# seungju-k1m/Distributed_RL

Hardware: NVIDIA H100
Metric: learner transitions/sec (sample+target+prio-update) (higher is better)
Workload: dtype f32

## Files before the change

distributed_rl_b200/csrc/common.cuh:

```cuda
#pragma once
#include <cuda_runtime.h>
#include <stdint.h>
#include <stdio.h>
#include <string.h>
#include <atomic>

#include "../../include/b2rl.h"

namespace b2rl {

void set_error(const char* fmt, ...);
extern std::atomic<int64_t> g_launches;
inline void count_launch(int n = 1) { g_launches.fetch_add(n, std::memory_order_relaxed); }

#define B2RL_CUDA(call)                                                              \
  do {                                                                               \
    cudaError_t e_ = (call);                                                         \
    if (e_ != cudaSuccess) {                                                         \
      b2rl::set_error("%s:%d %s -> %s", __FILE__, __LINE__, #call, cudaGetErrorString(e_)); \
      return B2RL_ERR_CUDA;                                                          \
    }                                                                                \
  } while (0)

#define B2RL_CHECK_LAUNCH()                                                          \
  do {                                                                               \
    cudaError_t e_ = cudaGetLastError();                                             \
    if (e_ != cudaSuccess) {                                                         \
      b2rl::set_error("%s:%d kernel launch -> %s", __FILE__, __LINE__, cudaGetErrorString(e_)); \
      return B2RL_ERR_CUDA;                                                          \
    }                                                                                \
  } while (0)

#define B2RL_REQUIRE(cond, msg)                                                      \
  do {                                                                               \
    if (!(cond)) {                                                                   \
      b2rl::set_error("%s:%d invalid argument: %s", __FILE__, __LINE__, msg);        \
      return B2RL_ERR_INVALID;                                                       \
    }                                                                                \
  } while (0)

struct DeviceGuard {
  int prev = -1;
  bool ok = true;
  explicit DeviceGuard(int dev) {
    if (cudaGetDevice(&prev) != cudaSuccess) { ok = false; return; }
    if (prev != dev && cudaSetDevice(dev) != cudaSuccess) ok = false;
    target = dev;
  }
  ~DeviceGuard() {
    if (prev >= 0 && prev != target) cudaSetDevice(prev);
  }
  int target = -1;
};

inline cudaError_t sm_count(int dev, int* out) {
  static int sms[64] = {0};
  if (!sms[dev & 63]) {
    const cudaError_t e = cudaDeviceGetAttribute(&sms[dev & 63], cudaDevAttrMultiProcessorCount, dev);
    if (e != cudaSuccess) return e;
  }
  *out = sms[dev & 63];
  return cudaSuccess;
}

template <auto K>
cudaError_t set_max_dynamic_smem(int dev, size_t bytes) {
  static bool done[64] = {false};
  if (done[dev & 63]) return cudaSuccess;
  const cudaError_t e = cudaFuncSetAttribute(K, cudaFuncAttributeMaxDynamicSharedMemorySize, (int)bytes);
  if (e == cudaSuccess) done[dev & 63] = true;
  return e;
}


__device__ __forceinline__ float powcr(float x, float e) {
  return (float)pow((double)x, (double)e);
}

__host__ __device__ __forceinline__ uint32_t lowbias32(uint32_t x) {
  x ^= x >> 16; x *= 0x7feb352dU; x ^= x >> 15; x *= 0x846ca68bU; x ^= x >> 16;
  return x;
}

__host__ __device__ __forceinline__ void philox4x32_10(uint64_t ctr, uint64_t seed, uint32_t out[4]) {
  uint32_t c0 = (uint32_t)ctr, c1 = (uint32_t)(ctr >> 32), c2 = 0u, c3 = 0u;
  uint32_t k0 = (uint32_t)seed, k1 = (uint32_t)(seed >> 32);
#pragma unroll
  for (int r = 0; r < 10; ++r) {
    uint64_t p0 = (uint64_t)0xD2511F53U * c0;
    uint64_t p1 = (uint64_t)0xCD9E8D57U * c2;
    uint32_t n0 = (uint32_t)(p1 >> 32) ^ c1 ^ k0;
    uint32_t n1 = (uint32_t)p1;
    uint32_t n2 = (uint32_t)(p0 >> 32) ^ c3 ^ k1;
    uint32_t n3 = (uint32_t)p0;
    c0 = n0; c1 = n1; c2 = n2; c3 = n3;
// ... 76 lines not shown
```

distributed_rl_b200/csrc/conv1.cu:

```cuda
#include "common.cuh"
#include "frames.cuh"
#include "hopper.cuh"

namespace b2rl {
namespace conv1 {

using namespace sm90;

constexpr int C_IN = 4, HW = 84, KS = 8, STRIDE = 4, OHW = 20;
constexpr int C_OUT_MAX = 32;
constexpr int K_TOTAL = C_IN * KS * KS;
constexpr int POS = OHW * OHW;
constexpr int TILE_M = 128;
constexpr int TILES = (POS + TILE_M - 1) / TILE_M;
constexpr int NSPLIT = 4;
constexpr int A_STAGES = 2;
constexpr int A_TILE_BYTES = TILE_M * K_TOTAL;
constexpr int A_CHUNK_BYTES = TILE_M * 128;
constexpr int RAW_STRIDE = 28288;
constexpr int CONSUMERS = 256, PRODUCERS = 256;
constexpr int THREADS = CONSUMERS + PRODUCERS + 32;

__host__ __device__ __forceinline__ int sw128_offset(int rows, int n, int k) {
  const int j = k >> 7, kk = k & 127;
// ... 47 lines not shown
struct Params {
  FrameSource src;
  const int64_t* idx;
  int64_t n;
  const int8_t* bq;
  const float* scale;
  float* out;
  int relu;
};

template <int N> struct Acc;
template <> struct Acc<128> {
  int32_t d[64];
  __device__ __forceinline__ void mma(uint64_t a, uint64_t b, uint32_t acc) { mma_u8s8_n128(d, a, b, acc); }
};
template <> struct Acc<64> {
  int32_t d[32];
  __device__ __forceinline__ void mma(uint64_t a, uint64_t b, uint32_t acc) { mma_u8s8_n64(d, a, b, acc); }
};

template <int N_NETS, int C_OUT, FrameKind KIND>
__global__ void __launch_bounds__(THREADS, 1)
k_conv1_fused(const __grid_constant__ Params P) {
  constexpr int N_PER_NET = NSPLIT * C_OUT;
  constexpr int N_TOTAL = N_NETS * N_PER_NET;
  constexpr int B_BYTES = N_TOTAL * K_TOTAL;
  extern __shared__ __align__(1024) uint8_t smem_raw[];
  uint8_t* smem = smem_raw + ((1024u - (sptr(smem_raw) & 1023u)) & 1023u);
  uint8_t* sB = smem;
  uint8_t* sA = smem + B_BYTES;
  uint8_t* sRaw = sA + A_STAGES * A_TILE_BYTES;
  __shared__ __align__(8) uint64_t b_full, raw_full[2], raw_empty[2], a_full[A_STAGES], a_empty[A_STAGES];
  __shared__ float s_scale[2 * C_OUT_MAX];
  if (threadIdx.x < N_NETS * C_OUT) s_scale[threadIdx.x] = P.scale[threadIdx.x] * (1.0f / 128.0f);

  const int warp = threadIdx.x >> 5, lane = threadIdx.x & 31;
  if (threadIdx.x == 0) {
    mbar_init(&b_full, 1);
    for (int i = 0; i < 2; ++i) { mbar_init(&raw_full[i], 1); mbar_init(&raw_empty[i], PRODUCERS); }
    for (int i = 0; i < A_STAGES; ++i) { mbar_init(&a_full[i], PRODUCERS); mbar_init(&a_empty[i], CONSUMERS); }
    mbar_init_fence();
  }
  __syncthreads();
  const int64_t units = P.n * TILES;
  const int64_t u0 = units * blockIdx.x / gridDim.x, u1 = units * (blockIdx.x + 1) / gridDim.x;
  const int64_t k_first = u0 / TILES, k_end = (u1 + TILES - 1) / TILES;

  if (warp == (CONSUMERS + PRODUCERS) / 32) {
    if (lane == 0) {
      const uint8_t* frames = frame_base<KIND>(P.src);
      mbar_expect_tx(&b_full, B_BYTES);
      constexpr int LOAD_CHUNK = (B_BYTES < 32768) ? B_BYTES : 32768;
      for (int off = 0; off < B_BYTES; off += LOAD_CHUNK) bulk_g2s(sB + off, P.bq + off, LOAD_CHUNK, &b_full);
      int it = 0;
      for (int64_t k = k_first; k < k_end; ++k, ++it) {
        const int s = it & 1;
        mbar_wait(&raw_empty[s], ((it >> 1) & 1) ^ 1);
        int64_t row = P.idx ? P.idx[k] : k;
        row = row < 0 ? 0 : (row >= P.src.rows ? P.src.rows - 1 : row);
        load_row<KIND>(P.src, frames, row, sRaw + s * RAW_STRIDE, &raw_full[s]);
      }
    }
  } else if (warp >= CONSUMERS / 32) {
    const int pt = threadIdx.x - CONSUMERS;
    const int r_local = pt & (TILE_M - 1);
    const int chalf = pt >> 7;
    int at = 0, it = 0;
    for (int64_t k = k_first; k < k_end; ++k, ++it) {
      const int s = it & 1;
      mbar_wait(&raw_full[s], (it >> 1) & 1);
      const uint8_t* raw = sRaw + s * RAW_STRIDE;
      const int t_lo = (int)max((int64_t)0, u0 - k * TILES), t_hi = (int)min((int64_t)TILES, u1 - k * TILES);
      for (int t = t_lo; t < t_hi; ++t, ++at) {
        const int stage = at % A_STAGES;
        mbar_wait(&a_empty[stage], ((at / A_STAGES) & 1) ^ 1);
// ... 99 lines not shown
  conv1::k_conv1_pack<<<c_out, conv1::K_TOTAL, 0, (cudaStream_t)stream>>>(w_dev, net, n_nets, c_out, bq_out_dev,
                                                                         scale_out_dev);
  count_launch();
  B2RL_CHECK_LAUNCH();
  return B2RL_OK;
}

extern "C" int b2rl_conv1_pack_jobs(const float* const* w_dev, const int32_t* net, const int32_t* n_nets,
                                    int8_t* const* bq_out_dev, float* const* scale_out_dev, int32_t jobs,
                                    int32_t c_out, void* stream) {
  B2RL_REQUIRE(w_dev && net && n_nets && bq_out_dev && scale_out_dev, "null argument");
  B2RL_REQUIRE(jobs >= 1 && jobs <= conv1::MAX_PACK_JOBS, "1..4 pack jobs");
  B2RL_REQUIRE(c_out == 16 || c_out == 32, "c_out must be 16 or 32");
  conv1::PackJobs J{};
  for (int j = 0; j < jobs; ++j) {
    B2RL_REQUIRE(w_dev[j] && bq_out_dev[j] && scale_out_dev[j], "null pack job");
    B2RL_REQUIRE(n_nets[j] >= 1 && n_nets[j] <= 2 && net[j] >= 0 && net[j] < n_nets[j], "n_nets must be 1 or 2");
    J.w[j] = w_dev[j]; J.bq[j] = bq_out_dev[j]; J.scale[j] = scale_out_dev[j];
    J.net[j] = net[j]; J.n_nets[j] = n_nets[j];
  }
  conv1::k_conv1_pack_jobs<<<dim3(c_out, jobs), conv1::K_TOTAL, 0, (cudaStream_t)stream>>>(J, c_out);
  count_launch();
  B2RL_CHECK_LAUNCH();
  return B2RL_OK;
}

template <int N_NETS, int C_OUT, FrameKind KIND>
static cudaError_t conv1_launch(const conv1::Params& P, unsigned grid, cudaStream_t st) {
  int dev = 0;
  cudaError_t e = cudaGetDevice(&dev);
  if (e == cudaSuccess)
    e = set_max_dynamic_smem<conv1::k_conv1_fused<N_NETS, C_OUT, KIND>>(dev, conv1::smem_bytes<N_NETS, C_OUT>());
  if (e != cudaSuccess) return e;
  conv1::k_conv1_fused<N_NETS, C_OUT, KIND><<<grid, conv1::THREADS, conv1::smem_bytes<N_NETS, C_OUT>(), st>>>(P);
  return cudaSuccess;
}

extern "C" int b2rl_conv1_fused(const b2rl_frames* frames, const int64_t* idx_dev, int64_t n, const int8_t* bq_dev,
                                const float* scale_dev, int32_t n_nets, int32_t c_out, float* out_dev, int32_t relu,
                                void* stream) {
  B2RL_REQUIRE(n >= 0, "negative n");
  conv1::Params P{};
  FrameKind kind;
  if (const int rc = check_frames(frames, P.src, kind)) return rc;
  if (n == 0) return B2RL_OK;
  B2RL_REQUIRE(bq_dev && scale_dev && out_dev, "null argument");
  B2RL_REQUIRE(n_nets == 1 || n_nets == 2, "n_nets must be 1 or 2");
  B2RL_REQUIRE(c_out == 16 || c_out == 32, "c_out must be 16 or 32");
  B2RL_REQUIRE(((uintptr_t)bq_dev % 16 == 0) && ((uintptr_t)out_dev % 16 == 0),
               "packed weights and output must be 16-byte aligned");
  int dev = 0;
  B2RL_CUDA(cudaGetDevice(&dev));
  int sms = 0;
  B2RL_CUDA(sm_count(dev, &sms));
  P.idx = idx_dev, P.n = n, P.bq = bq_dev, P.scale = scale_dev, P.out = out_dev, P.relu = relu;
  const int64_t units = n * conv1::TILES;
  const unsigned grid = (unsigned)((units < sms) ? units : sms);
  cudaStream_t st = (cudaStream_t)stream;
  const cudaError_t e = with_frame_kind(kind, [&](auto K) {
    constexpr FrameKind KIND = decltype(K)::value;
    if (c_out == 32) return n_nets == 1 ? conv1_launch<1, 32, KIND>(P, grid, st) : conv1_launch<2, 32, KIND>(P, grid, st);
    return n_nets == 1 ? conv1_launch<1, 16, KIND>(P, grid, st) : conv1_launch<2, 16, KIND>(P, grid, st);
  });
  B2RL_CUDA(e);
  count_launch();
  B2RL_CHECK_LAUNCH();
  return B2RL_OK;
}
```

distributed_rl_b200/csrc/dueling.cu:

```cuda
#include "common.cuh"

namespace b2rl {
namespace dueling {

constexpr int MAX_A = 32, MAX_H = 1024, ROWS_PER_CTA = 4;

__device__ __forceinline__ void load_weights(float* s_w, const float* __restrict__ wa, const float* __restrict__ wv,
                                             int A, int H) {
  const int na = (A * H) >> 2, nv = H >> 2;
  for (int i = threadIdx.x; i < na; i += blockDim.x)
    reinterpret_cast<float4*>(s_w)[i] = reinterpret_cast<const float4*>(wa)[i];
  for (int i = threadIdx.x; i < nv; i += blockDim.x)
    reinterpret_cast<float4*>(s_w + A * H)[i] = reinterpret_cast<const float4*>(wv)[i];
}

__device__ __forceinline__ float warp_sum(float v) {
#pragma unroll
  for (int o = 16; o > 0; o >>= 1) v = __fadd_rn(v, __shfl_xor_sync(0xffffffffu, v, o));
  return v;
}

constexpr int STAGE_UNROLL = 8;

template <int A_MAX>
__global__ void __launch_bounds__(ROWS_PER_CTA * 32)
k_dueling_forward(const float* __restrict__ h, int splits, int64_t split_stride, int M, int H,
                  const float* __restrict__ wa, int A, const float* __restrict__ wv, float* __restrict__ q,
                  float* __restrict__ h_out) {
  extern __shared__ float s_w[];
  float* s_h = s_w + A * H + H;
  load_weights(s_w, wa, wv, A, H);
  {
    const int m0 = blockIdx.x * ROWS_PER_CTA;
// ... 35 lines not shown
  float s[A_MAX], val = 0.0f;
#pragma unroll
  for (int j = 0; j < A_MAX; ++j) s[j] = 0.0f;
  for (int k = lane; k < H; k += 32) {
    const float ra = fmaxf(hr[k], 0.0f), rv = fmaxf(hr[H + k], 0.0f);
    val = __fmaf_rn(rv, s_w[A * H + k], val);
#pragma unroll
    for (int j = 0; j < A_MAX; ++j)
      if (j < A) s[j] = __fmaf_rn(ra, s_w[j * H + k], s[j]);
  }
#pragma unroll
  for (int o = 16; o > 0; o >>= 1) {
    val = __fadd_rn(val, __shfl_xor_sync(0xffffffffu, val, o));
#pragma unroll
    for (int j = 0; j < A_MAX; ++j)
      if (j < A) s[j] = __fadd_rn(s[j], __shfl_xor_sync(0xffffffffu, s[j], o));
  }
  float mine = 0.0f, total = 0.0f;
#pragma unroll
  for (int j = 0; j < A_MAX; ++j) {
    if (j < A) {
      total = __fadd_rn(total, s[j]);
      if (lane == j) mine = s[j];
    }
  }
  if (lane < A) q[(int64_t)m * A + lane] = __fsub_rn(__fadd_rn(mine, val), __fdiv_rn(total, (float)A));
}

__global__ void __launch_bounds__(ROWS_PER_CTA * 32)
k_dueling_backward_h(const float* __restrict__ h, const float* __restrict__ gq, int M, int H,
                     const float* __restrict__ wa, int A, const float* __restrict__ wv, float* __restrict__ gh,
                     float* __restrict__ ga) {
  extern __shared__ float s_w[];
  load_weights(s_w, wa, wv, A, H);
  __syncthreads();
  const int lane = threadIdx.x & 31, m = blockIdx.x * ROWS_PER_CTA + (threadIdx.x >> 5);
  if (m >= M) return;
  const float g = (lane < A) ? gq[(int64_t)m * A + lane] : 0.0f;
  const float gval = warp_sum(g);
  const float gadv = __fsub_rn(g, __fdiv_rn(gval, (float)A));
  if (lane < A) ga[(int64_t)m * (A + 1) + lane] = gadv;
  if (lane == 0) ga[(int64_t)m * (A + 1) + A] = gval;
  if (gh == nullptr) return;
  const float* hr = h + (int64_t)m * 2 * H;
  float* gr = gh + (int64_t)m * 2 * H;
  const int n = H >> 5;
  float ha[MAX_H / 32], hv[MAX_H / 32], s[MAX_H / 32];
#pragma unroll
  for (int i = 0; i < MAX_H / 32; ++i) {
    ha[i] = (i < n) ? hr[lane + 32 * i] : 0.0f;
    hv[i] = (i < n) ? hr[H + lane + 32 * i] : 0.0f;
    s[i] = 0.0f;
  }
  for (int j = 0; j < A; ++j) {
    const float gj = __shfl_sync(0xffffffffu, gadv, j);
#pragma unroll
    for (int i = 0; i < MAX_H / 32; ++i)
      if (i < n) s[i] = __fmaf_rn(gj, s_w[j * H + lane + 32 * i], s[i]);
  }
#pragma unroll
  for (int i = 0; i < MAX_H / 32; ++i) {
    if (i < n) {
      gr[lane + 32 * i] = ha[i] > 0.0f ? s[i] : 0.0f;
      gr[H + lane + 32 * i] = hv[i] > 0.0f ? __fmul_rn(gval, s_w[A * H + lane + 32 * i]) : 0.0f;
    }
  }
// ... 86 lines not shown
  if (A <= 8) {
    B2RL_CUDA(dueling_smem((const void*)dueling::k_dueling_forward<8>, smem));
    dueling::k_dueling_forward<8><<<grid, block, smem, st>>>(h_dev, splits, split_stride, (int)M, (int)H, wa_dev,
                                                                 (int)A, wv_dev, q_dev, h_out_dev);
  } else if (A <= 16) {
    B2RL_CUDA(dueling_smem((const void*)dueling::k_dueling_forward<16>, smem));
    dueling::k_dueling_forward<16><<<grid, block, smem, st>>>(h_dev, splits, split_stride, (int)M, (int)H, wa_dev,
                                                                 (int)A, wv_dev, q_dev, h_out_dev);
  } else {
    B2RL_CUDA(dueling_smem((const void*)dueling::k_dueling_forward<32>, smem));
    dueling::k_dueling_forward<32><<<grid, block, smem, st>>>(h_dev, splits, split_stride, (int)M, (int)H, wa_dev,
                                                                 (int)A, wv_dev, q_dev, h_out_dev);
  }
  count_launch();
  B2RL_CHECK_LAUNCH();
  return B2RL_OK;
}

extern "C" int b2rl_dueling_backward_w(const float* h_dev, const float* row_ws_dev, int64_t M, int64_t H, int64_t A,
                                       float* gwa_dev, float* gwv_dev, void* stream);

extern "C" int b2rl_dueling_backward(const float* h_dev, const float* gq_dev, int64_t M, int64_t H,
                                     const float* wa_dev, int64_t A, const float* wv_dev, float* gh_dev,
                                     float* gwa_dev, float* gwv_dev, float* row_ws_dev, void* stream) {
  if (int rc = dueling_check(h_dev, M, H, A)) return rc;
  B2RL_REQUIRE(gq_dev && wa_dev && wv_dev && row_ws_dev, "null argument");
  B2RL_REQUIRE(((uintptr_t)wa_dev % 16) == 0 && ((uintptr_t)wv_dev % 16) == 0, "weights must be 16-byte aligned");
  B2RL_REQUIRE((gwa_dev == nullptr) == (gwv_dev == nullptr), "both weight gradients or neither");
  cudaStream_t st = (cudaStream_t)stream;
  {
    const size_t smem = (size_t)(A + 1) * H * sizeof(float);
    B2RL_CUDA(dueling_smem((const void*)dueling::k_dueling_backward_h, smem));
    const unsigned grid = (unsigned)((M + dueling::ROWS_PER_CTA - 1) / dueling::ROWS_PER_CTA);
    dueling::k_dueling_backward_h<<<grid, dueling::ROWS_PER_CTA * 32, smem, st>>>(h_dev, gq_dev, (int)M, (int)H, wa_dev,
                                                                                 (int)A, wv_dev, gh_dev, row_ws_dev);
    count_launch();
    B2RL_CHECK_LAUNCH();
  }
  if (gwa_dev) return b2rl_dueling_backward_w(h_dev, row_ws_dev, M, H, A, gwa_dev, gwv_dev, stream);
  return B2RL_OK;
}

extern "C" int b2rl_dueling_backward_w(const float* h_dev, const float* row_ws_dev, int64_t M, int64_t H, int64_t A,
                                       float* gwa_dev, float* gwv_dev, void* stream) {
  if (int rc = dueling_check(h_dev, M, H, A)) return rc;
  B2RL_REQUIRE(row_ws_dev && gwa_dev && gwv_dev, "null argument");
  cudaStream_t st = (cudaStream_t)stream;
  {
    const unsigned grid = (unsigned)(2 * H / 8);
    if (A <= 8)
      dueling::k_dueling_backward_w<8><<<grid, 256, 0, st>>>(h_dev, row_ws_dev, (int)M, (int)H, (int)A, gwa_dev, gwv_dev);
    else if (A <= 16)
      dueling::k_dueling_backward_w<16><<<grid, 256, 0, st>>>(h_dev, row_ws_dev, (int)M, (int)H, (int)A, gwa_dev, gwv_dev);
    else
      dueling::k_dueling_backward_w<32><<<grid, 256, 0, st>>>(h_dev, row_ws_dev, (int)M, (int)H, (int)A, gwa_dev, gwv_dev);
    count_launch();
    B2RL_CHECK_LAUNCH();
  }
  return B2RL_OK;
}
```

distributed_rl_b200/csrc/hopper.cuh:

```cuda
#pragma once
#include <stdint.h>

namespace b2rl {
namespace sm90 {

__device__ __forceinline__ uint32_t sptr(const void* p) { return (uint32_t)__cvta_generic_to_shared(p); }
__device__ __forceinline__ void mbar_init(uint64_t* b, uint32_t c) {
  asm volatile("mbarrier.init.shared::cta.b64 [%0], %1;" ::"r"(sptr(b)), "r"(c));
}
__device__ __forceinline__ void mbar_init_fence() {
  asm volatile("fence.mbarrier_init.release.cluster;" ::: "memory");
  asm volatile("fence.proxy.async.shared::cta;" ::: "memory");
}
__device__ __forceinline__ void mbar_expect_tx(uint64_t* b, uint32_t bytes) {
  asm volatile("mbarrier.arrive.expect_tx.shared::cta.b64 _, [%0], %1;" ::"r"(sptr(b)), "r"(bytes) : "memory");
}
__device__ __forceinline__ void mbar_arrive(uint64_t* b) {
  asm volatile("mbarrier.arrive.shared::cta.b64 _, [%0];" ::"r"(sptr(b)) : "memory");
}
__device__ __forceinline__ void mbar_wait(uint64_t* b, uint32_t parity) {
  asm volatile(
      "{\n\t.reg .pred p;\n\t"
      "W_%=:\n\t"
      "mbarrier.try_wait.parity.shared::cta.b64 p, [%0], %1;\n\t"
      "@p bra D_%=;\n\t"
      "bra W_%=;\n\t"
      "D_%=:\n\t}" ::"r"(sptr(b)), "r"(parity) : "memory");
}
__device__ __forceinline__ void bulk_g2s(void* dst, const void* src, uint32_t bytes, uint64_t* bar) {
  asm volatile("cp.async.bulk.shared::cluster.global.mbarrier::complete_tx::bytes [%0], [%1], %2, [%3];" ::"r"(
                   sptr(dst)), "l"(src), "r"(bytes), "r"(sptr(bar)) : "memory");
}
__device__ __forceinline__ void bulk_s2g(void* dst, const void* src, uint32_t bytes) {
  asm volatile("cp.async.bulk.global.shared::cta.bulk_group [%0], [%1], %2;" ::"l"(dst), "r"(sptr(src)), "r"(bytes)
               : "memory");
}
__device__ __forceinline__ void bulk_commit() { asm volatile("cp.async.bulk.commit_group;" ::: "memory"); }
template <int N>
__device__ __forceinline__ void bulk_wait_read() { asm volatile("cp.async.bulk.wait_group.read %0;" ::"n"(N) : "memory"); }
__device__ __forceinline__ void bulk_wait_all() { asm volatile("cp.async.bulk.wait_group 0;" ::: "memory"); }
__device__ __forceinline__ void fence_async_smem() { asm volatile("fence.proxy.async.shared::cta;" ::: "memory"); }
__device__ __forceinline__ void named_sync(int id, int threads) {
  asm volatile("bar.sync %0, %1;" ::"r"(id), "r"(threads) : "memory");
}

__device__ __forceinline__ uint64_t make_desc(uint32_t smem_addr) {
  return (uint64_t)((smem_addr & 0x3FFFFu) >> 4) | (1ull << 16) | ((uint64_t)(1024 >> 4) << 32) | (1ull << 62);
}

__device__ __forceinline__ void wg_fence() { asm volatile("wgmma.fence.sync.aligned;" ::: "memory"); }
__device__ __forceinline__ void wg_commit() { asm volatile("wgmma.commit_group.sync.aligned;" ::: "memory"); }
template <int N>
__device__ __forceinline__ void wg_wait() { asm volatile("wgmma.wait_group.sync.aligned %0;" ::"n"(N) : "memory"); }
template <typename T, int R>
__device__ __forceinline__ void wg_fence_regs(T (&d)[R]) {
#pragma unroll
  for (int i = 0; i < R; ++i) asm volatile("" : "+r"(reinterpret_cast<uint32_t&>(d[i]))::"memory");
}

__device__ __forceinline__ void mma_tf32_n256(float (&d)[128], uint64_t a, uint64_t b, uint32_t accumulate) {
  asm volatile(
      "{\n\t.reg .pred p;\n\tsetp.ne.b32 p, %130, 0;\n\t"
      "wgmma.mma_async.sync.aligned.m64n256k8.f32.tf32.tf32 {%0,%1,%2,%3,%4,%5,%6,%7,%8,%9,%10,%11,%12,%13,%14,%15,%16,%17,%18,%19,%20,%21,%22,%23,%24,%25,%26,%27,%28,%29,%30,%31,%32,%33,%34,%35,%36,%37,%38,%39,%40,%41,%42,%43,%44,%45,%46,%47,%48,%49,%50,%51,%52,%53,%54,%55,%56,%57,%58,%59,%60,%61,%62,%63,%64,%65,%66,%67,%68,%69,%70,%71,%72,%73,%74,%75,%76,%77,%78,%79,%80,%81,%82,%83,%84,%85,%86,%87,%88,%89,%90,%91,%92,%93,%94,%95,%96,%97,%98,%99,%100,%101,%102,%103,%104,%105,%106,%107,%108,%109,%110,%111,%112,%113,%114,%115,%116,%117,%118,%119,%120,%121,%122,%123,%124,%125,%126,%127}, %128, %129, p, 1, 1;\n\t}"
      : "+f"(d[0]), "+f"(d[1]), "+f"(d[2]), "+f"(d[3]), "+f"(d[4]), "+f"(d[5]), "+f"(d[6]), "+f"(d[7]), "+f"(d[8]), "+f"(d[9]), "+f"(d[10]), "+f"(d[11]), "+f"(d[12]), "+f"(d[13]), "+f"(d[14]), "+f"(d[15]), "+f"(d[16]), "+f"(d[17]), "+f"(d[18]), "+f"(d[19]), "+f"(d[20]), "+f"(d[21]), "+f"(d[22]), "+f"(d[23]), "+f"(d[24]), "+f"(d[25]), "+f"(d[26]), "+f"(d[27]), "+f"(d[28]), "+f"(d[29]), "+f"(d[30]), "+f"(d[31]), "+f"(d[32]), "+f"(d[33]), "+f"(d[34]), "+f"(d[35]), "+f"(d[36]), "+f"(d[37]), "+f"(d[38]), "+f"(d[39]), "+f"(d[40]), "+f"(d[41]), "+f"(d[42]), "+f"(d[43]), "+f"(d[44]), "+f"(d[45]), "+f"(d[46]), "+f"(d[47]), "+f"(d[48]), "+f"(d[49]), "+f"(d[50]), "+f"(d[51]), "+f"(d[52]), "+f"(d[53]), "+f"(d[54]), "+f"(d[55]), "+f"(d[56]), "+f"(d[57]), "+f"(d[58]), "+f"(d[59]), "+f"(d[60]), "+f"(d[61]), "+f"(d[62]), "+f"(d[63]), "+f"(d[64]), "+f"(d[65]), "+f"(d[66]), "+f"(d[67]), "+f"(d[68]), "+f"(d[69]), "+f"(d[70]), "+f"(d[71]), "+f"(d[72]), "+f"(d[73]), "+f"(d[74]), "+f"(d[75]), "+f"(d[76]), "+f"(d[77]), "+f"(d[78]), "+f"(d[79]), "+f"(d[80]), "+f"(d[81]), "+f"(d[82]), "+f"(d[83]), "+f"(d[84]), "+f"(d[85]), "+f"(d[86]), "+f"(d[87]), "+f"(d[88]), "+f"(d[89]), "+f"(d[90]), "+f"(d[91]), "+f"(d[92]), "+f"(d[93]), "+f"(d[94]), "+f"(d[95]), "+f"(d[96]), "+f"(d[97]), "+f"(d[98]), "+f"(d[99]), "+f"(d[100]), "+f"(d[101]), "+f"(d[102]), "+f"(d[103]), "+f"(d[104]), "+f"(d[105]), "+f"(d[106]), "+f"(d[107]), "+f"(d[108]), "+f"(d[109]), "+f"(d[110]), "+f"(d[111]), "+f"(d[112]), "+f"(d[113]), "+f"(d[114]), "+f"(d[115]), "+f"(d[116]), "+f"(d[117]), "+f"(d[118]), "+f"(d[119]), "+f"(d[120]), "+f"(d[121]), "+f"(d[122]), "+f"(d[123]), "+f"(d[124]), "+f"(d[125]), "+f"(d[126]), "+f"(d[127])
      : "l"(a), "l"(b), "r"(accumulate));
}

__device__ __forceinline__ void mma_u8s8_n128(int32_t (&d)[64], uint64_t a, uint64_t b, uint32_t accumulate) {
  asm volatile(
      "{\n\t.reg .pred p;\n\tsetp.ne.b32 p, %66, 0;\n\t"
      "wgmma.mma_async.sync.aligned.m64n128k32.s32.u8.s8 {%0,%1,%2,%3,%4,%5,%6,%7,%8,%9,%10,%11,%12,%13,%14,%15,%16,%17,%18,%19,%20,%21,%22,%23,%24,%25,%26,%27,%28,%29,%30,%31,%32,%33,%34,%35,%36,%37,%38,%39,%40,%41,%42,%43,%44,%45,%46,%47,%48,%49,%50,%51,%52,%53,%54,%55,%56,%57,%58,%59,%60,%61,%62,%63}, %64, %65, p;\n\t}"
      : "+r"(d[0]), "+r"(d[1]), "+r"(d[2]), "+r"(d[3]), "+r"(d[4]), "+r"(d[5]), "+r"(d[6]), "+r"(d[7]), "+r"(d[8]), "+r"(d[9]), "+r"(d[10]), "+r"(d[11]), "+r"(d[12]), "+r"(d[13]), "+r"(d[14]), "+r"(d[15]), "+r"(d[16]), "+r"(d[17]), "+r"(d[18]), "+r"(d[19]), "+r"(d[20]), "+r"(d[21]), "+r"(d[22]), "+r"(d[23]), "+r"(d[24]), "+r"(d[25]), "+r"(d[26]), "+r"(d[27]), "+r"(d[28]), "+r"(d[29]), "+r"(d[30]), "+r"(d[31]), "+r"(d[32]), "+r"(d[33]), "+r"(d[34]), "+r"(d[35]), "+r"(d[36]), "+r"(d[37]), "+r"(d[38]), "+r"(d[39]), "+r"(d[40]), "+r"(d[41]), "+r"(d[42]), "+r"(d[43]), "+r"(d[44]), "+r"(d[45]), "+r"(d[46]), "+r"(d[47]), "+r"(d[48]), "+r"(d[49]), "+r"(d[50]), "+r"(d[51]), "+r"(d[52]), "+r"(d[53]), "+r"(d[54]), "+r"(d[55]), "+r"(d[56]), "+r"(d[57]), "+r"(d[58]), "+r"(d[59]), "+r"(d[60]), "+r"(d[61]), "+r"(d[62]), "+r"(d[63])
      : "l"(a), "l"(b), "r"(accumulate));
}

__device__ __forceinline__ void mma_u8s8_n64(int32_t (&d)[32], uint64_t a, uint64_t b, uint32_t accumulate) {
  asm volatile(
      "{\n\t.reg .pred p;\n\tsetp.ne.b32 p, %34, 0;\n\t"
// ... 8 lines not shown
```

distributed_rl_b200/csrc/optim.cu:

```cuda
#include "common.cuh"
#include "operand_image.cuh"

namespace b2rl {

constexpr int OPT_MAX_TENSORS = 24;
constexpr int OPT_THREADS = 256;
constexpr int OPT_PER_THREAD = 4;
constexpr int64_t OPT_CHUNK = (int64_t)OPT_THREADS * OPT_PER_THREAD;

struct OptTable {
  float* p[OPT_MAX_TENSORS];
  float* g[OPT_MAX_TENSORS];
  float* sq[OPT_MAX_TENSORS];
  float* ga[OPT_MAX_TENSORS];
  int64_t numel[OPT_MAX_TENSORS];
  int32_t block_start[OPT_MAX_TENSORS + 1];
  float* img_fwd[OPT_MAX_TENSORS];
  float* img_wt[OPT_MAX_TENSORS];
  int32_t cols[OPT_MAX_TENSORS];
  int32_t n_off[OPT_MAX_TENSORS];
  int32_t fwd_rows_pad[OPT_MAX_TENSORS], fwd_kc[OPT_MAX_TENSORS];
  int32_t wt_rows_pad[OPT_MAX_TENSORS], wt_kc[OPT_MAX_TENSORS];
  int32_t n_tensors;
};

__device__ __forceinline__ float rmsprop_elem(float p, float g, float& sq, float& ga, float lr, float alpha,
                                              float one_m_alpha, float eps, int centered) {
  sq = __fmaf_rn(one_m_alpha * g, g, sq * alpha);
  float avg;
  if (centered) {
    ga = __fmaf_rn(one_m_alpha, g - ga, ga);
    avg = __fsqrt_rn(__fmaf_rn(-ga, ga, sq));
  } else {
    avg = __fsqrt_rn(sq);
  }
  return p - lr * (g / (avg + eps));
}

__global__ void __launch_bounds__(OPT_THREADS)
k_rmsprop(const __grid_constant__ OptTable T, float lr, float alpha, float one_m_alpha, float eps, int centered,
          double* __restrict__ sumsq ) {
  __shared__ double s_part[OPT_THREADS / 32];
  int t = 0;
  while (t + 1 < T.n_tensors && (int)blockIdx.x >= T.block_start[t + 1]) ++t;
  const int64_t base = (int64_t)(blockIdx.x - T.block_start[t]) * OPT_CHUNK;
  const int64_t n = T.numel[t];
  float* __restrict__ P = T.p[t];
  float* __restrict__ G = T.g[t];
  float* __restrict__ SQ = T.sq[t];
  float* __restrict__ GA = T.ga[t];
  double acc = 0.0;
  if (T.img_fwd[t] || T.img_wt[t]) {
    __shared__ float tile[32][33];
    const int tiles_k = T.cols[t] / image::KC;
    const int bt = (int)(blockIdx.x - T.block_start[t]), rt = bt / tiles_k, kc = bt - rt * tiles_k;
    const int r = threadIdx.x >> 3, unit = threadIdx.x & 7;
    const int64_t i0 = (int64_t)(rt * 32 + r) * T.cols[t] + kc * image::KC + unit * 4;
    float4 p4 = *reinterpret_cast<const float4*>(P + i0);
    const float4 g4 = *reinterpret_cast<const float4*>(G + i0);
    float4 sq4 = *reinterpret_cast<const float4*>(SQ + i0);
    float4 ga4 = centered ? *reinterpret_cast<const float4*>(GA + i0) : make_float4(0.f, 0.f, 0.f, 0.f);
    float* pv = &p4.x;
    const float* gv = &g4.x;
    float* sqv = &sq4.x;
    float* gav = &ga4.x;
#pragma unroll
    for (int e = 0; e < 4; ++e) {
      pv[e] = rmsprop_elem(pv[e], gv[e], sqv[e], gav[e], lr, alpha, one_m_alpha, eps, centered);
      acc += (double)gv[e] * (double)gv[e];
    }
    *reinterpret_cast<float4*>(P + i0) = p4;
    *reinterpret_cast<float4*>(SQ + i0) = sq4;
    if (centered) *reinterpret_cast<float4*>(GA + i0) = ga4;
    *reinterpret_cast<float4*>(G + i0) = make_float4(0.f, 0.f, 0.f, 0.f);
    if (T.img_fwd[t]) {
// ... 11 lines not shown
      const int rows_pad = T.wt_rows_pad[t];
      image::store_unit(T.img_wt[t], image::offset(kc * image::KC + r, T.n_off[t] / image::KC + rt, unit, 256, rows_pad),
                        image::term_stride(T.wt_kc[t], rows_pad), v);
    }
  } else {
#pragma unroll
    for (int u = 0; u < OPT_PER_THREAD; ++u) {
      const int64_t i = base + (int64_t)u * OPT_THREADS + threadIdx.x;
      if (i < n) {
        const float g = G[i];
        float sq = SQ[i], ga = centered ? GA[i] : 0.0f;
        P[i] = rmsprop_elem(P[i], g, sq, ga, lr, alpha, one_m_alpha, eps, centered);
        SQ[i] = sq;
        if (centered) GA[i] = ga;
        G[i] = 0.0f;
        acc += (double)g * (double)g;
      }
    }
  }
  if (sumsq) {
#pragma unroll
    for (int o = 16; o > 0; o >>= 1) acc += __shfl_down_sync(0xffffffffu, acc, o);
    if ((threadIdx.x & 31) == 0) s_part[threadIdx.x >> 5] = acc;
    __syncthreads();
    if (threadIdx.x == 0) {
      double s = 0.0;
      for (int w = 0; w < OPT_THREADS / 32; ++w) s += s_part[w];
      atomicAdd(sumsq + t, s);
    }
  }
}

__global__ void k_grad_norm_finish(double* __restrict__ sumsq, int n, float* __restrict__ out) {
  if (threadIdx.x != 0 || blockIdx.x != 0) return;
  double s = 0.0;
  for (int i = 0; i < n; ++i) { s += sqrt(sumsq[i]); sumsq[i] = 0.0; }
  *out = (float)sqrt(s);
}

}

using namespace b2rl;

extern "C" int b2rl_rmsprop_step(float* const* params, float* const* grads, float* const* square_avg,
                                 float* const* grad_avg, const int64_t* numel, int32_t n_tensors, double lr,
                                 double alpha, double eps, int32_t centered, const int64_t* images,
                                 double* sumsq_scratch_dev, float* grad_norm_out_dev, void* stream) {
  B2RL_REQUIRE(n_tensors >= 1 && n_tensors <= OPT_MAX_TENSORS, "1..24 tensors");
  B2RL_REQUIRE(params && grads && square_avg && numel, "null argument");
  B2RL_REQUIRE(!centered || grad_avg, "centered RMSprop needs grad_avg");
  B2RL_REQUIRE(!grad_norm_out_dev || sumsq_scratch_dev,
               "the gradient norm needs a zero-initialised scratch of n_tensors doubles");
  OptTable T{};
  T.n_tensors = n_tensors;
  int64_t blocks = 0;
  for (int i = 0; i < n_tensors; ++i) {
    B2RL_REQUIRE(numel[i] >= 1 && params[i] && grads[i] && square_avg[i] && (!centered || grad_avg[i]),
                 "bad tensor entry");
    T.p[i] = params[i]; T.g[i] = grads[i]; T.sq[i] = square_avg[i]; T.ga[i] = centered ? grad_avg[i] : nullptr;
    T.numel[i] = numel[i];
    const int64_t* im = images ? images + 6 * i : nullptr;
    if (im && (im[0] || im[1])) {
      const int64_t rows = im[2], cols = im[3], total_n = im[4], n_off = im[5];
      B2RL_REQUIRE(rows >= 32 && cols >= 32 && rows % 32 == 0 && cols % 32 == 0 && rows * cols == numel[i] &&
                   n_off >= 0 && n_off % 32 == 0 && n_off + rows <= total_n && total_n < (1 << 30) &&
                   cols < (1 << 30), "image tensor: rows, cols and offsets must be multiples of 32 inside the stack");
      B2RL_REQUIRE(((uintptr_t)params[i] | (uintptr_t)grads[i] | (uintptr_t)square_avg[i] |
                    (uintptr_t)(centered ? grad_avg[i] : nullptr) | (uintptr_t)im[0] | (uintptr_t)im[1]) % 16 == 0,
                   "image tensor: 16-byte aligned arrays and images");
      T.img_fwd[i] = reinterpret_cast<float*>(im[0]);
      T.img_wt[i] = reinterpret_cast<float*>(im[1]);
      T.cols[i] = (int32_t)cols;
      T.n_off[i] = (int32_t)n_off;
      T.fwd_rows_pad[i] = (int32_t)((total_n + 255) / 256 * 256);
      T.fwd_kc[i] = (int32_t)(cols / image::KC);
      T.wt_rows_pad[i] = (int32_t)((cols + 255) / 256 * 256);
      T.wt_kc[i] = (int32_t)((total_n + image::KC - 1) / image::KC);
    }
    T.block_start[i] = (int32_t)blocks;
    blocks += (numel[i] + OPT_CHUNK - 1) / OPT_CHUNK;
  }
  T.block_start[n_tensors] = (int32_t)blocks;
  B2RL_REQUIRE(blocks < (1LL << 31), "too many elements");
  cudaStream_t st = (cudaStream_t)stream;
  k_rmsprop<<<(unsigned)blocks, OPT_THREADS, 0, st>>>(T, (float)lr, (float)alpha, (float)(1.0 - alpha), (float)eps,
                                                      centered, sumsq_scratch_dev);
  count_launch();
  if (grad_norm_out_dev) {
    k_grad_norm_finish<<<1, 32, 0, st>>>(sumsq_scratch_dev, n_tensors, grad_norm_out_dev);
    count_launch();
  }
  B2RL_CHECK_LAUNCH();
  return B2RL_OK;
}

extern "C" int b2rl_rmsprop_norm_finish(double* sumsq_scratch_dev, int32_t n_tensors, float* grad_norm_out_dev,
                                        void* stream) {
  B2RL_REQUIRE(sumsq_scratch_dev && grad_norm_out_dev, "null argument");
  B2RL_REQUIRE(n_tensors >= 1 && n_tensors <= OPT_MAX_TENSORS, "1..24 tensors");
  k_grad_norm_finish<<<1, 32, 0, (cudaStream_t)stream>>>(sumsq_scratch_dev, n_tensors, grad_norm_out_dev);
  count_launch();
  B2RL_CHECK_LAUNCH();
  return B2RL_OK;
}
```

distributed_rl_b200/csrc/targets.cu:

```cuda
#include "common.cuh"

#include <math.h>

namespace b2rl {

template <int THREADS>
__device__ __forceinline__ double block_sum(double v, double* s_buf) {
  const int lane = threadIdx.x & 31, warp = threadIdx.x >> 5;
#pragma unroll
  for (int o = 16; o > 0; o >>= 1) v += __shfl_down_sync(0xffffffffu, v, o);
  if (lane == 0) s_buf[warp] = v;
  __syncthreads();
  double r = 0.0;
  if (threadIdx.x == 0) {
    for (int w = 0; w < THREADS / 32; ++w) r += s_buf[w];
  }
  __syncthreads();
  return r;
}

constexpr int APEX_THREADS = 256;

__global__ void __launch_bounds__(APEX_THREADS)
k_apex_target(const float* __restrict__ q_s, const float* __restrict__ qn_on,
              const float* __restrict__ qn_tg, const int64_t* __restrict__ action,
              const float* __restrict__ reward, const float* __restrict__ notdone,
              const float* __restrict__ weight, int B, int A, float gamma_n, float alpha,
              float* __restrict__ target_out, float* __restrict__ td_out, float* __restrict__ prio_out,
              float* __restrict__ grad_q, float* __restrict__ scalars) {
  __shared__ double s_buf[APEX_THREADS / 32];
  double acc_loss = 0.0, acc_y = 0.0, acc_w = 0.0;
  for (int b = threadIdx.x; b < B; b += APEX_THREADS) {
    const float* qo = qn_on + (int64_t)b * A;
    int a_star = 0;
    float best = qo[0];
    for (int a = 1; a < A; ++a) {
      const float v = qo[a];
      if (v > best) { best = v; a_star = a; }
    }
    const float nxt = __fmul_rn(qn_tg[(int64_t)b * A + a_star], notdone[b]);
    const float y = __fadd_rn(reward[b], __fmul_rn(gamma_n, nxt));
    int a_b = (int)action[b];
    a_b = a_b < 0 ? 0 : (a_b >= A ? A - 1 : a_b);
    const float td_raw = __fsub_rn(y, q_s[(int64_t)b * A + a_b]);
    const float td = fminf(fmaxf(td_raw, -1.0f), 1.0f);
    const float w = weight[b];
    if (target_out) target_out[b] = y;
    if (td_out) td_out[b] = td;
    if (prio_out) prio_out[b] = powcr(__fadd_rn(fabsf(td), 1e-7f), alpha);
    if (grad_q) {
      const bool inside = (td_raw >= -1.0f) && (td_raw <= 1.0f);
      const float g = inside ? __fdiv_rn(-__fmul_rn(w, td), (float)B) : 0.0f;
      for (int a = 0; a < A; ++a) grad_q[(int64_t)b * A + a] = (a == a_b) ? g : 0.0f;
    }
    acc_loss += (double)__fmul_rn(w, __fmul_rn(td, td));
    acc_y += (double)y;
    acc_w += (double)w;
  }
  const double sl = block_sum<APEX_THREADS>(acc_loss, s_buf);
  const double sy = block_sum<APEX_THREADS>(acc_y, s_buf);
  const double sw = block_sum<APEX_THREADS>(acc_w, s_buf);
  if (threadIdx.x == 0 && scalars) {
    scalars[0] = __fmul_rn((float)(sl / (double)B), 0.5f);
// ... 209 lines not shown
```

distributed_rl_b200/csrc/tree.cu:

```cuda
#include "common.cuh"
#include "tree.cuh"

#include <math.h>
#include <stdlib.h>

namespace b2rl {

template <bool CG>
__device__ __forceinline__ float load_child_min(const TreeView& t, int k, int64_t node) {
  const int bits = (k == t.G) ? t.top_bits : 4;
  const float* p = (k == 1) ? t.leaf + (node << bits) : t.minv + t.off[k - 1] + (node << bits);
  float m = INFINITY;
  if (bits == 4) {
#pragma unroll
    for (int q = 0; q < 4; ++q) {
      const float4 v = ld4f<CG>(p + 4 * q);
      if (k == 1) {
        m = fminf(m, v.x > 0.0f ? v.x : INFINITY); m = fminf(m, v.y > 0.0f ? v.y : INFINITY);
        m = fminf(m, v.z > 0.0f ? v.z : INFINITY); m = fminf(m, v.w > 0.0f ? v.w : INFINITY);
      } else {
        m = fminf(fminf(m, v.x), fminf(v.y, fminf(v.z, v.w)));
      }
    }
  } else {
    for (int i = 0; i < (1 << bits); ++i) {
      const float v = CG ? __ldcg(p + i) : p[i];
      m = fminf(m, (k == 1 && !(v > 0.0f)) ? INFINITY : v);
    }
  }
  return m;
}

__device__ __forceinline__ double pairwise16(const double c[16]) {
// ... 92 lines not shown
#pragma unroll
        for (int i = 0; i < 16; ++i) { c[i] = s_sum2[i]; m3 = fminf(m3, s_min2[i]); }
        t.sum[t.off[3] + blockIdx.x] = pairwise16(c);
        t.minv[t.off[3] + blockIdx.x] = m3;
      }
    }
  }
  if (ticket == nullptr) return;
  __shared__ bool s_last;
  __threadfence();
  __syncthreads();
  if (tid == 0) {
    const unsigned int prev = atomicAdd(ticket, 1u);
    s_last = (prev == gridDim.x - 1);
    if (s_last) *ticket = 0u;
  }
  __syncthreads();
  if (!s_last) return;
  __threadfence();
  for (int k = fused_upto + 1; k <= t.G; ++k) {
    const int64_t nk = (k == t.G) ? 1 : (t.cap2 >> (4 * k));
    for (int64_t node = tid; node < nk; node += BUILD_THREADS) recompute_node<true>(t, k, node);
    __syncthreads();
  }
}

constexpr int SAMPLE_THREADS = 128;

__global__ void __launch_bounds__(SAMPLE_THREADS)
k_tree_sample(const __grid_constant__ TreeView t, const double* __restrict__ u01, uint64_t seed, uint64_t rng_offset,
              const uint64_t* __restrict__ rng_state, int64_t n, const float* __restrict__ n_valid_dev, float beta,
              const float* __restrict__ max_w_ext, int64_t* __restrict__ idx_out,
              float* __restrict__ prob_out, float* __restrict__ w_out, SmallFields small) {
  const int64_t k = (int64_t)blockIdx.x * SAMPLE_THREADS + threadIdx.x;
  if (rng_state) rng_stream_take(const_cast<uint64_t*>(rng_state), n, seed, rng_offset);
  if (k >= n) return;
  const double u = u01 ? u01[k] : philox_u01(seed, rng_offset + (uint64_t)k);
  double root, picked;
  const int64_t j = tree_draw(t, u, root, picked);
  idx_out[k] = j;
  fetch_small(small, j, k);
  if (prob_out == nullptr && w_out == nullptr) return;
  const float s32 = (float)root;
  const float p = (float)picked;
  const float prob = __fdiv_rn(p, s32);
  if (prob_out) prob_out[k] = prob;
  if (w_out) w_out[k] = is_weight(t, s32, prob, n_valid_dev, beta, max_w_ext);
}

__global__ void k_rng_seed(uint64_t* __restrict__ rng_state, uint64_t seed, uint64_t ctr) {
  rng_state[0] = seed; rng_state[1] = ctr; rng_state[2] = 0;
}

__global__ void k_philox_uniforms(uint64_t seed, uint64_t off, int64_t n, double* __restrict__ out) {
  const int64_t k = (int64_t)blockIdx.x * blockDim.x + threadIdx.x;
  if (k < n) out[k] = philox_u01(seed, off + (uint64_t)k);
}

__global__ void k_set_n_valid(float* __restrict__ n_valid_dev, float v) { *n_valid_dev = v; }

__global__ void k_tree_stats(const __grid_constant__ TreeView t, const float* __restrict__ n_valid_dev, float beta,
                             double* __restrict__ out, float* __restrict__ max_w_out) {
  const float n_valid = *n_valid_dev;
  const double root = t.sum[t.off[t.G]];
  const float s32 = (float)root;
  const float mn = t.minv[t.off[t.G]];
// ... 453 lines not shown
```

Before: 601,800.

## Use programmatic dependent launch to overlap kernel prologues across stages

Adds a launch helper that sets the programmatic stream serialization attribute, and inserts griddepcontrol wait and launch_dependents instructions into the sampling, targets, conv1, dueling-backward and optimizer kernels. Dependent kernels can now start their setup (barrier init, scheduling) while the previous kernel is still finishing, which hides launch latency between stages. The risk is a correctness hazard if any dependent kernel reads upstream outputs before its wait, and kernels launched without the attribute get no benefit.

```diff
diff --git a/distributed_rl_b200/csrc/common.cuh b/distributed_rl_b200/csrc/common.cuh
--- a/distributed_rl_b200/csrc/common.cuh
+++ b/distributed_rl_b200/csrc/common.cuh
@@ -4,6 +4,7 @@
 #include <stdio.h>
 #include <string.h>
 #include <atomic>
+#include <utility>
 
 #include "../../include/b2rl.h"
 
@@ -61,6 +62,25 @@
   }
   *out = sms[dev & 63];
   return cudaSuccess;
+}
+
+template <typename... KArgs, typename... Args>
+cudaError_t launch_dependent(void (*kernel)(KArgs...), dim3 grid, dim3 block, size_t smem, cudaStream_t st,
+                             Args&&... args) {
+  cudaLaunchAttribute attr[1];
+  attr[0].id = cudaLaunchAttributeProgrammaticStreamSerialization;
+  attr[0].val.programmaticStreamSerializationAllowed = 1;
+  cudaLaunchConfig_t cfg = {};
+  cfg.gridDim = grid;
+  cfg.blockDim = block;
+  cfg.dynamicSmemBytes = smem;
+  cfg.stream = st;
+  cfg.attrs = attr;
+  cfg.numAttrs = 1;
+  count_launch();
+  const cudaError_t e = cudaLaunchKernelEx(&cfg, kernel, std::forward<Args>(args)...);
+  if (e != cudaSuccess) cudaGetLastError();
+  return e;
 }
 
 template <auto K>
diff --git a/distributed_rl_b200/csrc/conv1.cu b/distributed_rl_b200/csrc/conv1.cu
--- a/distributed_rl_b200/csrc/conv1.cu
+++ b/distributed_rl_b200/csrc/conv1.cu
@@ -103,7 +103,6 @@
   uint8_t* sRaw = sA + A_STAGES * A_TILE_BYTES;
   __shared__ __align__(8) uint64_t b_full, raw_full[2], raw_empty[2], a_full[A_STAGES], a_empty[A_STAGES];
   __shared__ float s_scale[2 * C_OUT_MAX];
-  if (threadIdx.x < N_NETS * C_OUT) s_scale[threadIdx.x] = P.scale[threadIdx.x] * (1.0f / 128.0f);
 
   const int warp = threadIdx.x >> 5, lane = threadIdx.x & 31;
   if (threadIdx.x == 0) {
@@ -112,6 +111,9 @@
     for (int i = 0; i < A_STAGES; ++i) { mbar_init(&a_full[i], PRODUCERS); mbar_init(&a_empty[i], CONSUMERS); }
     mbar_init_fence();
   }
+  grid_dependency_wait();
+  launch_dependents();
+  if (threadIdx.x < N_NETS * C_OUT) s_scale[threadIdx.x] = P.scale[threadIdx.x] * (1.0f / 128.0f);
   __syncthreads();
   const int64_t units = P.n * TILES;
   const int64_t u0 = units * blockIdx.x / gridDim.x, u1 = units * (blockIdx.x + 1) / gridDim.x;
@@ -277,8 +279,8 @@
   if (e == cudaSuccess)
     e = set_max_dynamic_smem<conv1::k_conv1_fused<N_NETS, C_OUT, KIND>>(dev, conv1::smem_bytes<N_NETS, C_OUT>());
   if (e != cudaSuccess) return e;
-  conv1::k_conv1_fused<N_NETS, C_OUT, KIND><<<grid, conv1::THREADS, conv1::smem_bytes<N_NETS, C_OUT>(), st>>>(P);
-  return cudaSuccess;
+  return launch_dependent(conv1::k_conv1_fused<N_NETS, C_OUT, KIND>, grid, conv1::THREADS,
+                          conv1::smem_bytes<N_NETS, C_OUT>(), st, P);
 }
 
 extern "C" int b2rl_conv1_fused(const b2rl_frames* frames, const int64_t* idx_dev, int64_t n, const int8_t* bq_dev,
@@ -308,7 +310,5 @@
     return n_nets == 1 ? conv1_launch<1, 16, KIND>(P, grid, st) : conv1_launch<2, 16, KIND>(P, grid, st);
   });
   B2RL_CUDA(e);
-  count_launch();
-  B2RL_CHECK_LAUNCH();
   return B2RL_OK;
 }
diff --git a/distributed_rl_b200/csrc/dueling.cu b/distributed_rl_b200/csrc/dueling.cu
--- a/distributed_rl_b200/csrc/dueling.cu
+++ b/distributed_rl_b200/csrc/dueling.cu
@@ -1,4 +1,5 @@
 #include "common.cuh"
+#include "hopper.cuh"
 
 namespace b2rl {
 namespace dueling {
@@ -100,6 +101,7 @@
                      const float* __restrict__ wa, int A, const float* __restrict__ wv, float* __restrict__ gh,
                      float* __restrict__ ga) {
   extern __shared__ float s_w[];
+  sm90::grid_dependency_wait();
   load_weights(s_w, wa, wv, A, H);
   __syncthreads();
   const int lane = threadIdx.x & 31, m = blockIdx.x * ROWS_PER_CTA + (threadIdx.x >> 5);
@@ -252,10 +254,8 @@
     const size_t smem = (size_t)(A + 1) * H * sizeof(float);
     B2RL_CUDA(dueling_smem((const void*)dueling::k_dueling_backward_h, smem));
     const unsigned grid = (unsigned)((M + dueling::ROWS_PER_CTA - 1) / dueling::ROWS_PER_CTA);
-    dueling::k_dueling_backward_h<<<grid, dueling::ROWS_PER_CTA * 32, smem, st>>>(h_dev, gq_dev, (int)M, (int)H, wa_dev,
-                                                                                 (int)A, wv_dev, gh_dev, row_ws_dev);
-    count_launch();
-    B2RL_CHECK_LAUNCH();
+    B2RL_CUDA(launch_dependent(dueling::k_dueling_backward_h, grid, dueling::ROWS_PER_CTA * 32, smem, st, h_dev, gq_dev,
+                               (int)M, (int)H, wa_dev, (int)A, wv_dev, gh_dev, row_ws_dev));
   }
   if (gwa_dev) return b2rl_dueling_backward_w(h_dev, row_ws_dev, M, H, A, gwa_dev, gwv_dev, stream);
   return B2RL_OK;
diff --git a/distributed_rl_b200/csrc/hopper.cuh b/distributed_rl_b200/csrc/hopper.cuh
--- a/distributed_rl_b200/csrc/hopper.cuh
+++ b/distributed_rl_b200/csrc/hopper.cuh
@@ -44,6 +44,9 @@
   asm volatile("bar.sync %0, %1;" ::"r"(id), "r"(threads) : "memory");
 }
 
+__device__ __forceinline__ void grid_dependency_wait() { asm volatile("griddepcontrol.wait;" ::: "memory"); }
+__device__ __forceinline__ void launch_dependents() { asm volatile("griddepcontrol.launch_dependents;" ::: "memory"); }
+
 __device__ __forceinline__ uint64_t make_desc(uint32_t smem_addr) {
   return (uint64_t)((smem_addr & 0x3FFFFu) >> 4) | (1ull << 16) | ((uint64_t)(1024 >> 4) << 32) | (1ull << 62);
 }
diff --git a/distributed_rl_b200/csrc/optim.cu b/distributed_rl_b200/csrc/optim.cu
--- a/distributed_rl_b200/csrc/optim.cu
+++ b/distributed_rl_b200/csrc/optim.cu
@@ -1,4 +1,5 @@
 #include "common.cuh"
+#include "hopper.cuh"
 #include "operand_image.cuh"
 
 namespace b2rl {
@@ -41,6 +42,7 @@
 k_rmsprop(const __grid_constant__ OptTable T, float lr, float alpha, float one_m_alpha, float eps, int centered,
           double* __restrict__ sumsq ) {
   __shared__ double s_part[OPT_THREADS / 32];
+  sm90::launch_dependents();
   int t = 0;
   while (t + 1 < T.n_tensors && (int)blockIdx.x >= T.block_start[t + 1]) ++t;
   const int64_t base = (int64_t)(blockIdx.x - T.block_start[t]) * OPT_CHUNK;
@@ -118,6 +120,7 @@
 }
 
 __global__ void k_grad_norm_finish(double* __restrict__ sumsq, int n, float* __restrict__ out) {
+  sm90::grid_dependency_wait();
   if (threadIdx.x != 0 || blockIdx.x != 0) return;
   double s = 0.0;
   for (int i = 0; i < n; ++i) { s += sqrt(sumsq[i]); sumsq[i] = 0.0; }
@@ -172,11 +175,9 @@
   k_rmsprop<<<(unsigned)blocks, OPT_THREADS, 0, st>>>(T, (float)lr, (float)alpha, (float)(1.0 - alpha), (float)eps,
                                                       centered, sumsq_scratch_dev);
   count_launch();
-  if (grad_norm_out_dev) {
-    k_grad_norm_finish<<<1, 32, 0, st>>>(sumsq_scratch_dev, n_tensors, grad_norm_out_dev);
-    count_launch();
-  }
   B2RL_CHECK_LAUNCH();
+  if (grad_norm_out_dev)
+    B2RL_CUDA(launch_dependent(k_grad_norm_finish, 1, 32, 0, st, sumsq_scratch_dev, n_tensors, grad_norm_out_dev));
   return B2RL_OK;
 }
 
@@ -184,8 +185,7 @@
                                         void* stream) {
   B2RL_REQUIRE(sumsq_scratch_dev && grad_norm_out_dev, "null argument");
   B2RL_REQUIRE(n_tensors >= 1 && n_tensors <= OPT_MAX_TENSORS, "1..24 tensors");
-  k_grad_norm_finish<<<1, 32, 0, (cudaStream_t)stream>>>(sumsq_scratch_dev, n_tensors, grad_norm_out_dev);
-  count_launch();
-  B2RL_CHECK_LAUNCH();
+  B2RL_CUDA(launch_dependent(k_grad_norm_finish, 1, 32, 0, (cudaStream_t)stream, sumsq_scratch_dev, n_tensors,
+                             grad_norm_out_dev));
   return B2RL_OK;
 }
diff --git a/distributed_rl_b200/csrc/targets.cu b/distributed_rl_b200/csrc/targets.cu
--- a/distributed_rl_b200/csrc/targets.cu
+++ b/distributed_rl_b200/csrc/targets.cu
@@ -1,4 +1,5 @@
 #include "common.cuh"
+#include "hopper.cuh"
 
 #include <math.h>
 
@@ -29,6 +30,7 @@
               float* __restrict__ target_out, float* __restrict__ td_out, float* __restrict__ prio_out,
               float* __restrict__ grad_q, float* __restrict__ scalars) {
   __shared__ double s_buf[APEX_THREADS / 32];
+  sm90::launch_dependents();
   double acc_loss = 0.0, acc_y = 0.0, acc_w = 0.0;
   for (int b = threadIdx.x; b < B; b += APEX_THREADS) {
     const float* qo = qn_on + (int64_t)b * A;
diff --git a/distributed_rl_b200/csrc/tree.cu b/distributed_rl_b200/csrc/tree.cu
--- a/distributed_rl_b200/csrc/tree.cu
+++ b/distributed_rl_b200/csrc/tree.cu
@@ -1,4 +1,5 @@
 #include "common.cuh"
+#include "hopper.cuh"
 #include "tree.cuh"
 
 #include <math.h>
@@ -157,6 +158,7 @@
               const uint64_t* __restrict__ rng_state, int64_t n, const float* __restrict__ n_valid_dev, float beta,
               const float* __restrict__ max_w_ext, int64_t* __restrict__ idx_out,
               float* __restrict__ prob_out, float* __restrict__ w_out, SmallFields small) {
+  sm90::launch_dependents();
   const int64_t k = (int64_t)blockIdx.x * SAMPLE_THREADS + threadIdx.x;
   if (rng_state) rng_stream_take(const_cast<uint64_t*>(rng_state), n, seed, rng_offset);
   if (k >= n) return;
```

Result: no change. 602,500 (median of 6 runs) (+0.1%).
